# mvenouziou/Boosted_DETR

Hardware: AMD Instinct MI355X
Metric: images/sec training step (fwd+matcher+loss+bwd), 640x640 N=100 (higher is better)
Workload: dtype f32 (conv/GEMM products as 3 split-f16 [fwd] / split-bf16 [grad] MFMA products, f32 accumulate)

## Files before the change

### boosted_detr_amd/csrc/gemm_common.h

```cpp
#pragma once
#include "common.h"
#include <type_traits>

namespace bdgemm {

enum { ST_STORE = 0, ST_ACCUM = 1, ST_ATOMIC = 2 };
enum { AR_FP32 = 0, AR_BF16X3 = 1, AR_FP16X3 = 2, AR_P16_F16 = 3, AR_P16_BF16 = 4, AR_BF16X6 = 5 };

struct GemmParams {
    int I, J, R;
    int nb1;
    int splitk, r_chunk;
    int tiles_i, tiles_j;
    float* c; int64_t ldc, sc0, sc1;
    const float* bias; float alpha; int act; int mode;
    float* stat_sum; float* stat_sq;
    int vec_store;
    int rowmap;
    int rm_OW, rm_OHOW, rm_H, rm_W, rm_stride;
    int rm_off;
    int ngroups;
    const float* ga[4]; const float* gb[4]; float* gc[4]; const float* gbias[4]; int gI[4];
    const float* bnb_y; const float* bnb_mean; const float* bnb_rstd; const float* bnb_gamma; const float* bnb_beta;
    int bnb_relu; float* bnb_sum_g; float* bnb_sum_gx;
    const unsigned long long* bnb_mask;
    const float* bnb2_y; const float* bnb2_mean; const float* bnb2_rstd; float* bnb2_sum_gx;
    const unsigned long long* acc_mask;
    const float* acc_src; int acc_H, acc_W;
    int b_f16;
#ifdef BDETR_SGEMM_DIAG
    int dbg;
#endif
};

#ifdef BDETR_SGEMM_DIAG
#define BDETR_DBG(g, bits) (((g).dbg & (bits)) != 0)
#else
#define BDETR_DBG(g, bits) false
#endif

inline void init_params(GemmParams& g) {
    g = GemmParams{};
    g.nb1 = 1; g.splitk = 1; g.alpha = 1.f; g.mode = ST_STORE;
}

__device__ __forceinline__ float apply_act(float v, int act) {
    if (act == BDETR_ACT_RELU) return fmaxf(v, 0.f);
    if (act == BDETR_ACT_TANH) return tanhf(v);
    return v;
}

__device__ __forceinline__ int xcd_tile(int bid, int nwg) {
    const int q = nwg >> 3, r = nwg & 7, xcd = bid & 7, idx = bid >> 3;
    return (xcd < r ? xcd * (q + 1) : r * (q + 1) + (xcd - r) * q) + idx;
}

template <int BM, int BN, int WM, int WN>
__device__ __forceinline__ void gemm_load_bias(const GemmParams& g, int j0, float (&bias_pre)[BN / WN / 32]) {
    const int tid = threadIdx.x, lane = tid & 63, wave = tid >> 6, wn = wave % WN;
#pragma unroll
    for (int b = 0; b < BN / WN / 32; ++b) {
        const int j = j0 + wn * (BN / WN) + b * 32 + (lane & 31);
        bias_pre[b] = (g.bias != nullptr && j < g.J) ? g.bias[j] : 0.f;
    }
}

template <int BM, int BN, int WM, int WN>
__device__ __forceinline__ void gemm_bias_act_stats(f32x16 (&acc)[BM / WM / 32][BN / WN / 32], const GemmParams& g, int tile_i, int i0, int j0,
                                                    const float* bias_pre = nullptr) {
    constexpr int WTM = BM / WM, WTN = BN / WN, TM = WTM / 32, TN = WTN / 32;
    int tid = threadIdx.x;
    asm volatile("" : "+v"(tid));
    const int lane = tid & 63, wave = __builtin_amdgcn_readfirstlane(tid >> 6);
    const int wm = wave / WN, wn = wave % WN, li = lane & 31, lh = lane >> 5;
    auto bias_act_stats = [&](auto act_c) {
        constexpr int ACT = decltype(act_c)::value;
#pragma unroll
        for (int b = 0; b < TN; ++b) {
            const int j = j0 + wn * WTN + b * 32 + li;
            const bool jok = j < g.J;
            const float bias = bias_pre != nullptr ? bias_pre[b] : ((g.bias != nullptr && jok) ? g.bias[j] : 0.f);
            float csum = 0.f, csq = 0.f;
#pragma unroll
            for (int a = 0; a < TM; ++a) {
#pragma unroll
                for (int e = 0; e < 16; ++e) {
                    const int i = i0 + wm * WTM + a * 32 + (e & 3) + 8 * (e >> 2) + 4 * lh;
                    const float v = apply_act(g.alpha * acc[a][b][e] + bias, ACT);
                    acc[a][b][e] = v;
                    const float vs = (i < g.I && jok) ? v : 0.f;
                    csum += vs; csq += vs * vs;
                }
            }
            if (g.stat_sum != nullptr) {
                csum += __shfl_xor(csum, 32, 64);
                csq += __shfl_xor(csq, 32, 64);
                if (lh == 0 && jok) {
                    const int64_t chunk = (int64_t)tile_i * WM + wm;
                    g.stat_sum[chunk * g.J + j] = csum;
                    g.stat_sq[chunk * g.J + j] = csq;
                }
            }
        }
    };
    if (g.act == BDETR_ACT_NONE) {
        if (g.bias != nullptr || g.alpha != 1.f || g.stat_sum != nullptr) bias_act_stats(std::integral_constant<int, BDETR_ACT_NONE>{});
    } else if (g.act == BDETR_ACT_RELU) bias_act_stats(std::integral_constant<int, BDETR_ACT_RELU>{});
    else bias_act_stats(std::integral_constant<int, BDETR_ACT_TANH>{});
}

__device__ __forceinline__ unsigned mask_bits4(const unsigned long long* mask, int64_t i) {
    const unsigned long long* w = mask + (i >> 6) * 4;
    const int b = (int)(i & 63);
    return (unsigned)((w[0] >> b) & 1ull) | ((unsigned)((w[1] >> b) & 1ull) << 1) | ((unsigned)((w[2] >> b) & 1ull) << 2) | ((unsigned)((w[3] >> b) & 1ull) << 3);
}

template <int BM, int BN, int WM, int WN, int NT, int LDS_FLOATS, bool MASKED_VARIANTS = false, bool BNB2_ONLY = false, bool COMPACT_ONLY = false>
__device__ __forceinline__ void gemm_epilogue(f32x16 (&acc)[BM / WM / 32][BN / WN / 32], const GemmParams& g, float* lds,
                                              int tile_i, int i0, int j0, float* cbase, const float* bias_pre = nullptr) {
    constexpr int WTM = BM / WM, WTN = BN / WN, TM = WTM / 32, TN = WTN / 32;
    const int tid = threadIdx.x, lane = tid & 63, wave = tid >> 6;
    const int wm = wave / WN, wn = wave % WN, li = lane & 31, lh = lane >> 5;
    auto out_row = [&](int i) -> int64_t {
        if (!g.rowmap) return i;
        int n = i / g.rm_OHOW; int rem = i - n * g.rm_OHOW;
        int oh = rem / g.rm_OW; int ow = rem - oh * g.rm_OW;
        return ((int64_t)n * g.rm_H + (int64_t)oh * g.rm_stride) * g.rm_W + (int64_t)ow * g.rm_stride + g.rm_off;
    };
    gemm_bias_act_stats<BM, BN, WM, WN>(acc, g, tile_i, i0, j0, bias_pre);

    if (g.vec_store && g.mode != ST_ATOMIC) {
        constexpr bool PAD = BM * (BN + 4) <= LDS_FLOATS;
        constexpr int CLD = PAD ? BN + 4 : BN;
        static_assert(BM * CLD <= LDS_FLOATS, "epilogue tile must fit in the staging LDS");
        constexpr bool SWZ = !PAD && BN % 64 == 0;
        __syncthreads();
#pragma unroll
        for (int a = 0; a < TM; ++a)
#pragma unroll
            for (int b = 0; b < TN; ++b)
#pragma unroll
                for (int e = 0; e < 16; ++e)
                    lds[(wm * WTM + a * 32 + (e & 3) + 8 * (e >> 2) + 4 * lh) * CLD + ((wn * WTN + b * 32 + li) ^ (SWZ ? lh << 5 : 0))] = acc[a][b][e];
        __syncthreads();
        constexpr int V_PER_ROW = BN / 4, RSTEP = NT / V_PER_ROW, ITERS = BM / RSTEP;
        static_assert(NT % V_PER_ROW == 0 && BM % RSTEP == 0, "a thread keeps one column group and a fixed row stride");
        static_assert(!SWZ || RSTEP % 8 == 0, "the swizzle bit of a thread's rows must not change between iterations");
        const int c4 = tid % V_PER_ROW, r0 = tid / V_PER_ROW;
        const int jc = j0 + 4 * c4;
        const bool jok = jc < g.J;
        const float* lrow = lds + r0 * CLD + ((4 * c4) ^ (SWZ ? ((r0 >> 2) & 1) << 5 : 0));
        auto vec_out = [&](auto rowmap_c, auto accum_c, auto bnb_c, auto masked_c, auto bnb2_c, auto compact_c) {
            constexpr bool ROWMAP = decltype(rowmap_c)::value, ACCUM = decltype(accum_c)::value, BNB = decltype(bnb_c)::value, MASKED = decltype(masked_c)::value;
            constexpr bool BNB2 = decltype(bnb2_c)::value;
            constexpr bool COMPACT = decltype(compact_c)::value;
            static_assert(!COMPACT || (ACCUM && MASKED && !ROWMAP && !BNB2), "the compact old gradient rides the masked accumulate");
            static_assert(!BNB2 || (BNB && ACCUM && MASKED), "the second BatchNorm rides the masked accumulate with masked sums");
            constexpr int NPART = (ACCUM && BNB) ? (BNB2 && ITERS % 4 == 0 ? 4 : 2) : 1, PIT = ITERS / NPART;
            static_assert(ITERS % NPART == 0, "the tile splits into equal parts");
            f32x4 bnv[BNB ? 6 : 1];
            f32x4 bn2[BNB2 ? 3 : 1];
            if constexpr (BNB2) {
                bn2[0] = f32x4{0, 0, 0, 0}; bn2[1] = f32x4{0, 0, 0, 0}; bn2[2] = f32x4{0, 0, 0, 0};
                if (jok) { bn2[0] = *reinterpret_cast<const f32x4*>(g.bnb2_mean + jc); bn2[1] = *reinterpret_cast<const f32x4*>(g.bnb2_rstd + jc); }
            }
            if constexpr (BNB) {
#pragma unroll
                for (int q = 0; q < 6; ++q) bnv[q] = f32x4{0, 0, 0, 0};
                if (jok) {
                    bnv[0] = *reinterpret_cast<const f32x4*>(g.bnb_mean + jc); bnv[1] = *reinterpret_cast<const f32x4*>(g.bnb_rstd + jc);
                    bnv[2] = *reinterpret_cast<const f32x4*>(g.bnb_gamma + jc); bnv[3] = *reinterpret_cast<const f32x4*>(g.bnb_beta + jc);
                }
            }
#pragma unroll
// ... 145 lines not shown
```

### boosted_detr_amd/csrc/sgemm.hip

```cpp
#include "gemm_common.h"
#include "p16.h"
#include <stdlib.h>
#include <string.h>
#include <type_traits>
#include <utility>

using namespace bdgemm;

namespace {

constexpr int BK = 32;
constexpr unsigned OOB = 0xFFFFFFF0u;
constexpr unsigned NUM_RECORDS = 0xFFFFFF00u;

typedef __bf16 bf16x8 __attribute__((ext_vector_type(8)));
typedef _Float16 f16x8 __attribute__((ext_vector_type(8)));
typedef unsigned int u32x4 __attribute__((ext_vector_type(4)));
typedef unsigned int u32x2 __attribute__((ext_vector_type(2)));
typedef short s16x4 __attribute__((ext_vector_type(4)));
typedef __attribute__((address_space(3))) void lds_void;

__device__ __forceinline__ __amdgpu_buffer_rsrc_t make_rsrc(const void* p, unsigned records = NUM_RECORDS) {
    const unsigned long long a = reinterpret_cast<unsigned long long>(p);
    const unsigned lo = __builtin_amdgcn_readfirstlane((unsigned)a), hi = __builtin_amdgcn_readfirstlane((unsigned)(a >> 32));
// ... 63 lines not shown
    static __device__ __forceinline__ Col col(const Op& op, int x0, int slot, int x_lim, int r_uni, int lane_row) {
        const int r_first = r_uni + lane_row;
        Col c; c.ok = x0 + 8 * (slot >> 1) < x_lim; c.r = r_first;
        c.off = (unsigned)r_first * op.ld * 4u + (unsigned)x0 * 4u + 16u * (unsigned)slot; return c;
    }
    template <int RPI> static __device__ __forceinline__ unsigned voff(const Op&, const Col& c, int r_lim) { return (c.ok && c.r < r_lim) ? c.off : OOB; }
    static __device__ __forceinline__ void advance(const Op& op, Col& c) { c.r += BK; c.off += (unsigned)BK * op.ld * 4u; }
};
struct XXPatch {
    using Op = PPatch;
    using Row = int; using Step = int;
    static __device__ __forceinline__ unsigned records(const Op&) { return NUM_RECORDS; }
    struct Col { int r, oh, ow, ih, iw; unsigned off; bool ok; };
    static __device__ __forceinline__ Col col(const Op& op, int x0, int slot, int x_lim, int r_uni, int lane_row) {
        const int r_first = r_uni + lane_row;
        Col c; const int x = x0 + 8 * (slot >> 1);
        c.ok = x < x_lim; c.r = r_first;
        const int tap = x / op.C, ch = x - tap * op.C;
        const int tr = tap / op.S, ts = tap - tr * op.S;
        const int ohw = op.OH * op.OW;
        const int n = r_first / ohw, rem = r_first - n * ohw;
        c.oh = rem / op.OW; c.ow = rem - c.oh * op.OW;
        c.ih = c.oh * op.stride - op.pad + tr; c.iw = c.ow * op.stride - op.pad + ts;
        c.off = ((unsigned)(n * op.H * op.W) + (unsigned)(c.ih * op.W + c.iw)) * (unsigned)op.C * 4u + (unsigned)ch * 4u + 16u * (unsigned)(slot & 1);
        return c;
    }
    template <int RPI> static __device__ __forceinline__ unsigned voff(const Op& op, const Col& c, int r_lim) {
        const bool ok = c.ok && c.r < r_lim && (unsigned)c.ih < (unsigned)op.H && (unsigned)c.iw < (unsigned)op.W;
        return ok ? c.off : OOB;
    }
    static __device__ __forceinline__ void advance(const Op& op, Col& c) {
        c.r += BK;
        c.ow += op.d_ow; c.oh += op.d_oh; c.iw += op.d_ow * op.stride; c.ih += op.d_oh * op.stride; c.off += op.k_step;
        const bool w = c.ow >= op.OW;
        c.ow -= w ? op.OW : 0; c.oh += w ? 1 : 0; c.iw -= w ? op.OW * op.stride : 0; c.ih += w ? op.stride : 0; c.off += w ? op.k_wrap_ow : 0u;
        if (op.single_wrap) {
            const bool v = c.oh >= op.OH;
            c.oh -= v ? op.OH : 0; c.ih -= v ? op.OH * op.stride : 0; c.off += v ? op.k_wrap_oh : 0u;
        } else {
            while (c.oh >= op.OH) { c.oh -= op.OH; c.ih -= op.OH * op.stride; c.off += op.k_wrap_oh; }
        }
    }
};

__device__ __forceinline__ int xx_swz(int r) { return ((r & 1) << 3) | ((r >> 1) & 1); }

#if defined(BDETR_SGEMM_STAMPS) && defined(BDETR_SGEMM_DIAG)
__device__ unsigned long long g_stamps[64];
#endif

constexpr int lds_bytes_for(int bm, int bn, int ns) { return ns * (bm + bn) * 128 > bm * bn * 4 ? ns * (bm + bn) * 128 : bm * bn * 4; }

enum { EPI_PLAIN = 0, EPI_ROWMAP = 1, EPI_VEC = 8, EPI_BNB2 = 16, EPI_COMPACT = 32 };
template <int BM, int BN, int WM, int WN, bool STATS = true, int EPI = EPI_ROWMAP>
__device__ __forceinline__ void direct_epilogue(f32x16 (&acc)[BM / WM / 32][BN / WN / 32], const GemmParams& g, int tile_i, int i0, int j0, const float* bias_pre) {
    constexpr int WTM = BM / WM, WTN = BN / WN, TM = WTM / 32, TN = WTN / 32;
    constexpr unsigned FAR = 0x80000000u;
    if constexpr (STATS) gemm_bias_act_stats<BM, BN, WM, WN>(acc, g, tile_i, i0, j0, bias_pre);
    int tid = threadIdx.x;
    asm volatile("" : "+v"(tid));
    const int lane = tid & 63, wave = __builtin_amdgcn_readfirstlane(tid >> 6);
    const int wm = wave / WN, wn = wave % WN, li = lane & 31, lh = lane >> 5;

    const unsigned ldc4 = (unsigned)g.ldc * 4u;
    const int rows_here = min(BM, g.I - i0);
    const int jl = j0 + wn * WTN + li;
    auto tile_rsrc = [&](const float* base) {
        const unsigned long long p = reinterpret_cast<unsigned long long>(base) + (unsigned long long)i0 * ldc4;
        const unsigned lo = __builtin_amdgcn_readfirstlane((unsigned)p), hi = __builtin_amdgcn_readfirstlane((unsigned)(p >> 32));
        return __builtin_amdgcn_make_buffer_rsrc(reinterpret_cast<void*>(((unsigned long long)hi << 32) | lo), 0,
                                                 __builtin_amdgcn_readfirstlane(rows_here * (int)ldc4), 0x00020000);
    };
    unsigned vcol[TN];
#pragma unroll
    for (int b = 0; b < TN; ++b) vcol[b] = jl + b * 32 < g.J ? (unsigned)(wm * WTM + 4 * lh) * ldc4 + (unsigned)(jl + b * 32) * 4u : FAR;
    auto for_rows = [&](auto&& f) {
        unsigned ro = 0;
#pragma unroll
        for (int a = 0; a < TM; ++a)
#pragma unroll
            for (int e = 0; e < 16; ++e) { f(a, e, ro); ro += (e & 3) == 3 ? 5u * ldc4 : ldc4; }
    };

    if constexpr ((EPI & EPI_ROWMAP) != 0) if (g.rowmap) {
        const __amdgpu_buffer_rsrc_t rsC = make_rsrc(g.c);
        const int i = i0 + wm * WTM + (lane % WTM);
        const int n = i / g.rm_OHOW, rem = i - n * g.rm_OHOW, oh = rem / g.rm_OW, ow = rem - oh * g.rm_OW;
        const unsigned rmap = i < g.I ? (unsigned)((n * g.rm_H + oh * g.rm_stride) * g.rm_W + ow * g.rm_stride + g.rm_off) * ldc4 : OOB;
        const bool accum = g.mode == ST_ACCUM;
#pragma unroll
        for (int a = 0; a < TM; ++a)
#pragma unroll
            for (int e = 0; e < 16; ++e) {
                const unsigned ro = (unsigned)__shfl((int)rmap, a * 32 + (e & 3) + 8 * (e >> 2) + 4 * lh, 64);
#pragma unroll
                for (int b = 0; b < TN; ++b) {
                    const unsigned vo = (ro != OOB && jl + b * 32 < g.J) ? ro + (unsigned)(jl + b * 32) * 4u : OOB;
                    float v = acc[a][b][e];
                    if (accum) v += __uint_as_float(__builtin_amdgcn_raw_buffer_load_b32(rsC, vo, 0, 0));
                    if (!BDETR_DBG(g, 1)) __builtin_amdgcn_raw_buffer_store_b32(__float_as_uint(v), rsC, vo, 0, 0);
                }
            }
        return;
    }

    const __amdgpu_buffer_rsrc_t rsC = tile_rsrc(g.c);
// ... 2 lines not shown
#pragma unroll
        for (int b = 0; b < TN; ++b) {
            const float v = acc[a][b][e];
            __builtin_amdgcn_raw_buffer_store_b32(__float_as_uint(v), rsC, vcol[b] + ro, 0, 0);
        }
    });
}

template <int BM, int BN, int WM, int WN>
__device__ __forceinline__ void atomic_epilogue(f32x16 (&acc)[BM / WM / 32][BN / WN / 32], const GemmParams& g, int i0, int j0) {
    constexpr int WTM = BM / WM, WTN = BN / WN, TM = WTM / 32, TN = WTN / 32;
    constexpr unsigned FAR = 0x80000000u;
    const int tid = threadIdx.x, lane = tid & 63, wave = __builtin_amdgcn_readfirstlane(tid >> 6);
    const int wm = wave / WN, wn = wave % WN, li = lane & 31, lh = lane >> 5;
    const unsigned ldc4 = (unsigned)g.ldc * 4u;
    const int rows_here = min(BM, g.I - i0);
    const unsigned long long p = reinterpret_cast<unsigned long long>(g.c) + (unsigned long long)i0 * ldc4;
    const unsigned lo = __builtin_amdgcn_readfirstlane((unsigned)p), hi = __builtin_amdgcn_readfirstlane((unsigned)(p >> 32));
    const __amdgpu_buffer_rsrc_t rsC = __builtin_amdgcn_make_buffer_rsrc(reinterpret_cast<void*>(((unsigned long long)hi << 32) | lo), 0,
                                                                         __builtin_amdgcn_readfirstlane(rows_here * (int)ldc4), 0x00020000);
    unsigned vcol[TN];
#pragma unroll
    for (int b = 0; b < TN; ++b) {
        const int j = j0 + wn * WTN + b * 32 + li;
        vcol[b] = j < g.J ? (unsigned)(wm * WTM + 4 * lh) * ldc4 + (unsigned)j * 4u : FAR;
    }
    unsigned ro = 0;
#pragma unroll
    for (int a = 0; a < TM; ++a)
#pragma unroll
        for (int e = 0; e < 16; ++e) {
#pragma unroll
            for (int b = 0; b < TN; ++b) {
                const float v = g.alpha * acc[a][b][e];
                __builtin_amdgcn_raw_ptr_buffer_atomic_fadd_f32(v, rsC, vcol[b] + ro, 0, 0);
            }
            ro += (e & 3) == 3 ? 5u * ldc4 : ldc4;
            asm volatile("" : "+v"(ro));
        }
}

constexpr int default_occ(int bm, int bn, int wm, int wn, int ns) { return (wm * wn == 4 && 2 * lds_bytes_for(bm, bn, ns) <= 160 * 1024) ? 2 : (wm * wn == 8 ? 2 : 1); }

template <int BM, int BN, int WM, int WN, int NS, class LA, class LB, bool XX, bool F16, bool PP = false, int OCC = default_occ(BM, BN, WM, WN, NS), int EPI = EPI_ROWMAP>
__global__ __launch_bounds__(WM * WN * 64, OCC)
void sgemm_kernel(typename LA::Op opa, typename LB::Op opb, GemmParams g)
{
    constexpr int NW = WM * WN, NT = NW * 64;
    constexpr int WTM = BM / WM, WTN = BN / WN, TM = WTM / 32, TN = WTN / 32;
    static_assert(TM >= 1 && TN >= 1, "wave tile must hold at least one 32x32 MFMA tile");
    constexpr int A_BYTES = BM * 128, B_BYTES = BN * 128, STAGE_BYTES = A_BYTES + B_BYTES;
    constexpr int NIA = A_BYTES / 1024 / NW, NIB = B_BYTES / 1024 / NW;
    static_assert(NIA >= 1 && NIB >= 1 && NIA * NW * 1024 == A_BYTES && NIB * NW * 1024 == B_BYTES, "tile / wave count mismatch");
    constexpr int LDS_BYTES = lds_bytes_for(BM, BN, NS);
    static_assert(NS >= 2 && NS <= 4 && LDS_BYTES <= 160 * 1024, "LDS budget");
    static_assert(BK == 32, "fragment helpers assume two 16-deep MFMA steps per stage");
    __shared__ __attribute__((aligned(16))) unsigned char lds[LDS_BYTES];

    const int tid = threadIdx.x;
    const int lane = tid & 63;
    const int wave = __builtin_amdgcn_readfirstlane(tid >> 6);
    const int wm = wave / WN, wn = wave % WN;
    const int li = lane & 31, lh = lane >> 5;

    constexpr bool PERSIST = !PP && !XX && std::is_same_v<LA, RRDense> && (EPI & EPI_VEC) == 0;
    static_assert(PP ? (NS == 3 && NW == 8) : NS == 2, "the plain loops are written for a two-stage ring, the ping-pong loop for three stages and 8 waves");
    const int nwg = g.tiles_i * g.tiles_j;
    const int total = PERSIST ? nwg : nwg * (int)gridDim.z;
    int vb = PERSIST ? (int)blockIdx.x : (int)(blockIdx.z * nwg + blockIdx.x);
    int tile_i, i0, j0, zz;
    auto locate = [&](int v) {
        const int lin = xcd_tile(v, total);
        zz = lin / nwg;
        const int wg = lin - zz * nwg;
        tile_i = wg / g.tiles_j;
        const int tile_j = wg - tile_i * g.tiles_j;
        i0 = tile_i * BM; j0 = tile_j * BN;
    };
    locate(vb);

    int r_begin = 0, r_end = g.R;
    if (g.splitk > 1) { r_begin = zz * g.r_chunk; r_end = min(g.R, r_begin + g.r_chunk); }

    const __amdgpu_buffer_rsrc_t rsA = make_rsrc(opa.p, LA::records(opa));
    const __amdgpu_buffer_rsrc_t rsB = make_rsrc(opb.p, LB::records(opb));

    typename LA::Row rowA[NIA]; typename LB::Row rowB[NIB]; typename LA::Col colA[NIA]; typename LB::Col colB[NIB];
    int rrA[NIA], rrB[NIB];
    static_assert(XX || NW % 2 == 0, "one source chunk per lane needs an even wave count");
    const int qsrc = (lane & 7) ^ (((wave & 1) << 2) | (lane >> 4));
    const int klimA = min(r_end, (int)opa.cols) - 8 * (qsrc >> 1), klimB = min(r_end, (int)opb.cols) - 8 * (qsrc >> 1);
    typename LA::Step stA; typename LB::Step stB;
    auto setup_rows = [&]() {
        if constexpr (!XX) {
#pragma unroll
            for (int t = 0; t < NIA; ++t) {
                const int x = (t * NW + wave) * 8 + (lane >> 3);
                rowA[t] = LA::row(opa, i0 + x, qsrc);
            }
#pragma unroll
            for (int t = 0; t < NIB; ++t) {
                const int x = (t * NW + wave) * 8 + (lane >> 3);
                rowB[t] = LB::row(opb, j0 + x, qsrc);
            }
            stA = LA::step_init(opa, r_begin); stB = LB::step_init(opb, r_begin);
        }
    };
    setup_rows();
    if constexpr (XX) {
        constexpr int SA = BM / 4, SB = BN / 4;
        static_assert(SA >= 16 && SB >= 16 && SA <= 64 && SB <= 64, "XX tiles: 64 <= BX <= 256");
#pragma unroll
        for (int t = 0; t < NIA; ++t) {
            const int ru = (t * NW + wave) * (64 / SA), r = ru + lane / SA;
            rrA[t] = r;
            colA[t] = LA::col(opa, i0, (lane % SA) ^ xx_swz(r), opa.cols, r_begin + ru, lane / SA);
        }
#pragma unroll
        for (int t = 0; t < NIB; ++t) {
            const int ru = (t * NW + wave) * (64 / SB), r = ru + lane / SB;
            rrB[t] = r;
            colB[t] = LB::col(opb, j0, (lane % SB) ^ xx_swz(r), opb.cols, r_begin + ru, lane / SB);
        }
    }

    auto issue_one = [&](int buf, int r0, auto l_c) {
        constexpr int l = decltype(l_c)::value;
        unsigned char* sa = lds + buf * STAGE_BYTES;
        if constexpr (l < NIA) {
            constexpr int t = l;
            unsigned vo;
            if constexpr (!XX) vo = LA::voff(opa, rowA[t], stA, r0, klimA);
            else               vo = LA::template voff<256 / BM>(opa, colA[t], min(r_end, opa.rows));
            __builtin_amdgcn_raw_ptr_buffer_load_lds(rsA, (lds_void*)(sa + (t * NW + wave) * 1024), 16, (int)vo, 0, 0, 0);
        } else {
            constexpr int t = l - NIA;
            unsigned vo;
            if constexpr (!XX) vo = LB::voff(opb, rowB[t], stB, r0, klimB);
            else               vo = LB::template voff<256 / BN>(opb, colB[t], min(r_end, opb.rows));
            __builtin_amdgcn_raw_ptr_buffer_load_lds(rsB, (lds_void*)(sa + A_BYTES + (t * NW + wave) * 1024), 16, (int)vo, 0, 0, 0);
        }
    };
    constexpr int NLOAD = NIA + NIB;
    auto issue_all = [&](int buf, int r0) {
        if (BDETR_DBG(g, 16)) return;
        [&]<int... L>(std::integer_sequence<int, L...>) { (issue_one(buf, r0, std::integral_constant<int, L>{}), ...); }(std::make_integer_sequence<int, NLOAD>{});
        if constexpr (!XX) { LA::step_next(opa, stA); LB::step_next(opb, stB); }
        else {
#pragma unroll
            for (int t = 0; t < NIA; ++t) LA::advance(opa, colA[t]);
#pragma unroll
            for (int t = 0; t < NIB; ++t) LB::advance(opb, colB[t]);
        }
    };

    f32x16 acc[TM][TN];
    auto zero_acc = [&]() {
        float z = 0.f;
        asm volatile("" : "+v"(z));
#pragma unroll
        for (int a = 0; a < TM; ++a)
#pragma unroll
            for (int b = 0; b < TN; ++b)
#pragma unroll
                for (int e = 0; e < 16; ++e) acc[a][b][e] = z;
    };
    zero_acc();

    auto frag_rr = [&](const unsigned char* tile, int x, int ks, u32x4& hi, u32x4& lo) {
        const int s = (2 * (2 * ks + lh)) ^ ((x >> 1) & 7);
        const unsigned char* p = tile + x * 128;
        hi = *reinterpret_cast<const u32x4*>(p + s * 16);
        lo = *reinterpret_cast<const u32x4*>(p + (s ^ 1) * 16);
    };
    auto frag_xx = [&](const unsigned char* tile, auto rowbytes_c, int xw, auto ks_c, u32x4& hi, u32x4& lo) {
        constexpr int rowbytes = decltype(rowbytes_c)::value, ks = decltype(ks_c)::value;
        const int g16 = (lane >> 4) & 1, q = (lane >> 2) & 3, p = lane & 3;
        const int unit = (xw + 16 * g16 + 4 * p) >> 3;
        const int r0 = 8 * lh + q;
        const int sl = (2 * unit) ^ xx_swz(r0);
        const unsigned base = (unsigned)(size_t)(__attribute__((address_space(3))) const unsigned char*)tile + (unsigned)(r0 * rowbytes + 8 * (p & 1));
        const unsigned ah = base + (unsigned)(sl * 16), al = base + (unsigned)((sl ^ 1) * 16);
        u32x2 h0, h1, l0, l1;
        constexpr int o0 = ks * 16 * rowbytes, o1 = o0 + 4 * rowbytes;
        static_assert(o1 < 65536, "ds offset field");
        asm volatile("ds_read_b64_tr_b16 %0, %1 offset:%2" : "=v"(h0) : "v"(ah), "n"(o0));
        asm volatile("ds_read_b64_tr_b16 %0, %1 offset:%2" : "=v"(l0) : "v"(al), "n"(o0));
        asm volatile("ds_read_b64_tr_b16 %0, %1 offset:%2" : "=v"(h1) : "v"(ah), "n"(o1));
        asm volatile("ds_read_b64_tr_b16 %0, %1 offset:%2" : "=v"(l1) : "v"(al), "n"(o1));
        hi[0] = h0[0]; hi[1] = h0[1]; hi[2] = h1[0]; hi[3] = h1[1];
        lo[0] = l0[0]; lo[1] = l0[1]; lo[2] = l1[0]; lo[3] = l1[1];
    };
    auto frag_wait = [&](u32x4 (&ah)[TM], u32x4 (&al)[TM], u32x4 (&bh)[TN], u32x4 (&bl)[TN]) {
        if constexpr (XX) {
            static_assert(TM <= 2 && TN <= 2, "frag_wait ties at most 2 + 2 fragments");
            if constexpr (TM == 2 && TN == 2)
                asm volatile("s_waitcnt lgkmcnt(0)" : "+v"(ah[0]), "+v"(al[0]), "+v"(ah[1]), "+v"(al[1]), "+v"(bh[0]), "+v"(bl[0]), "+v"(bh[1]), "+v"(bl[1]));
            else if constexpr (TM == 2 && TN == 1)
                asm volatile("s_waitcnt lgkmcnt(0)" : "+v"(ah[0]), "+v"(al[0]), "+v"(ah[1]), "+v"(al[1]), "+v"(bh[0]), "+v"(bl[0]));
            else if constexpr (TM == 1 && TN == 2)
                asm volatile("s_waitcnt lgkmcnt(0)" : "+v"(ah[0]), "+v"(al[0]), "+v"(bh[0]), "+v"(bl[0]), "+v"(bh[1]), "+v"(bl[1]));
            else
                asm volatile("s_waitcnt lgkmcnt(0)" : "+v"(ah[0]), "+v"(al[0]), "+v"(bh[0]), "+v"(bl[0]));
        }
    };
    auto load_frags = [&](int buf, auto ks_c, u32x4 (&ah)[TM], u32x4 (&al)[TM], u32x4 (&bh)[TN], u32x4 (&bl)[TN]) {
        constexpr int ks = decltype(ks_c)::value;
        const unsigned char* tA = lds + buf * STAGE_BYTES;
        const unsigned char* tB = tA + A_BYTES;
#pragma unroll
        for (int a = 0; a < TM; ++a) {
            if constexpr (!XX) frag_rr(tA, wm * WTM + a * 32 + li, ks, ah[a], al[a]);
            else               frag_xx(tA, std::integral_constant<int, BM * 4>{}, wm * WTM + a * 32, ks_c, ah[a], al[a]);
        }
#pragma unroll
        for (int b = 0; b < TN; ++b) {
            if constexpr (!XX) frag_rr(tB, wn * WTN + b * 32 + li, ks, bh[b], bl[b]);
            else               frag_xx(tB, std::integral_constant<int, BN * 4>{}, wn * WTN + b * 32, ks_c, bh[b], bl[b]);
        }
    };
    auto mfma_ks = [&](const u32x4 (&ah)[TM], const u32x4 (&al)[TM], const u32x4 (&bh)[TN], const u32x4 (&bl)[TN]) {
#pragma unroll
        for (int a = 0; a < TM; ++a)
#pragma unroll
            for (int b = 0; b < TN; ++b) {
                if constexpr (F16) {
#define H8(v) __builtin_bit_cast(f16x8, v)
                    acc[a][b] = __builtin_amdgcn_mfma_f32_32x32x16_f16(H8(al[a]), H8(bh[b]), acc[a][b], 0, 0, 0);
                    acc[a][b] = __builtin_amdgcn_mfma_f32_32x32x16_f16(H8(ah[a]), H8(bl[b]), acc[a][b], 0, 0, 0);
                    acc[a][b] = __builtin_amdgcn_mfma_f32_32x32x16_f16(H8(ah[a]), H8(bh[b]), acc[a][b], 0, 0, 0);
#undef H8
                } else {
#define BF8(v) __builtin_bit_cast(bf16x8, v)
                    acc[a][b] = __builtin_amdgcn_mfma_f32_32x32x16_bf16(BF8(al[a]), BF8(bh[b]), acc[a][b], 0, 0, 0);
                    acc[a][b] = __builtin_amdgcn_mfma_f32_32x32x16_bf16(BF8(ah[a]), BF8(bl[b]), acc[a][b], 0, 0, 0);
                    acc[a][b] = __builtin_amdgcn_mfma_f32_32x32x16_bf16(BF8(ah[a]), BF8(bh[b]), acc[a][b], 0, 0, 0);
#undef BF8
                }
            }
    };
    auto f16pair_to_bf16pair = [&](u32x4& hi, u32x4& lo) {
        const unsigned hw[4] = {hi[0], hi[1], hi[2], hi[3]}, lw[4] = {lo[0], lo[1], lo[2], lo[3]};
#pragma unroll
        for (int w = 0; w < 4; ++w) {
            const p16_f32x2 hf = __builtin_convertvector(__builtin_bit_cast(p16_f16x2, hw[w]), p16_f32x2);
            const p16_f32x2 lf = __builtin_convertvector(__builtin_bit_cast(p16_f16x2, lw[w]), p16_f32x2);
            unsigned bh_, bl_;
            p16_split2_bf16(hf[0] + lf[0], hf[1] + lf[1], bh_, bl_);
            hi[w] = bh_; lo[w] = bl_;
        }
    };
    auto kstep = [&](int buf) {
        if (BDETR_DBG(g, 8)) return;
        auto half = [&](auto ks_c) {
            u32x4 ah[TM], al[TM], bh[TN], bl[TN];
            load_frags(buf, ks_c, ah, al, bh, bl);
            frag_wait(ah, al, bh, bl);
            if constexpr (XX && !F16) {
                if (g.b_f16) {
#pragma unroll
                    for (int b = 0; b < TN; ++b) f16pair_to_bf16pair(bh[b], bl[b]);
                }
            }
            mfma_ks(ah, al, bh, bl);
        };
        static_assert(BK / 16 == 2, "two 16-deep halves per stage");
        half(std::integral_constant<int, 0>{});
        half(std::integral_constant<int, 1>{});
    };

    if constexpr (PP) {
        constexpr int NLOAD_ = NIA + NIB;
        const int nk = (r_end - r_begin + BK - 1) / BK;
        float bias_pre[TN];
        gemm_load_bias<BM, BN, WM, WN>(g, j0, bias_pre);
        const bool grpY = wave >= NW / 2;
        u32x4 fah[2][TM], fal[2][TM], fbh[2][TN], fbl[2][TN];
        auto read_all = [&](auto buf_c) {
            constexpr int buf = decltype(buf_c)::value;
            load_frags(buf, std::integral_constant<int, 0>{}, fah[0], fal[0], fbh[0], fbl[0]);
            load_frags(buf, std::integral_constant<int, 1>{}, fah[1], fal[1], fbh[1], fbl[1]);
            frag_wait(fah[0], fal[0], fbh[0], fbl[0]);
            frag_wait(fah[1], fal[1], fbh[1], fbl[1]);
            if constexpr (XX && !F16) {
                if (g.b_f16) {
#pragma unroll
                    for (int ks = 0; ks < 2; ++ks)
#pragma unroll
                        for (int b = 0; b < TN; ++b) f16pair_to_bf16pair(fbh[ks][b], fbl[ks][b]);
                }
            }
        };
        auto mfma_step = [&]() {
            asm volatile("s_waitcnt lgkmcnt(0)" ::: "memory");
            __builtin_amdgcn_sched_barrier(0);
            __builtin_amdgcn_s_setprio(1);
#pragma unroll
            for (int ks = 0; ks < 2; ++ks) mfma_ks(fah[ks], fal[ks], fbh[ks], fbl[ks]);
            __builtin_amdgcn_s_setprio(0);
            __builtin_amdgcn_sched_barrier(0);
        };
        if (nk > 0) issue_all(0, r_begin);
        if (nk > 1) issue_all(1, r_begin + BK);
        if (nk > 1) asm volatile("s_waitcnt vmcnt(%0)\n\ts_barrier" :: "n"(NLOAD_) : "memory");
        else        asm volatile("s_waitcnt vmcnt(0)\n\ts_barrier" ::: "memory");
        if (!grpY) read_all(std::integral_constant<int, 0>{});
        auto step = [&](int t, auto b0_c, auto b1_c, auto b2_c) {
            constexpr int b2 = decltype(b2_c)::value;
            if (!grpY) {
                mfma_step();
                asm volatile("s_waitcnt vmcnt(0)\n\ts_barrier" ::: "memory");
            } else {
                read_all(b0_c);
                if (t + 2 < nk) {
                    issue_all(b2, r_begin + (t + 2) * BK);
                    asm volatile("s_waitcnt vmcnt(%0)\n\ts_barrier" :: "n"(NLOAD_) : "memory");
                } else {
                    asm volatile("s_waitcnt vmcnt(0)\n\ts_barrier" ::: "memory");
                }
            }
            if (grpY) {
                mfma_step();
            } else {
                if (t + 1 < nk) read_all(b1_c);
                if (t + 2 < nk) issue_all(b2, r_begin + (t + 2) * BK);
            }
            asm volatile("s_barrier" ::: "memory");
        };
        using I0 = std::integral_constant<int, 0>; using I1 = std::integral_constant<int, 1>; using I2 = std::integral_constant<int, 2>;
        for (int t = 0; t < nk; t += 3) {
            step(t, I0{}, I1{}, I2{});
            if (t + 1 < nk) step(t + 1, I1{}, I2{}, I0{});
            if (t + 2 < nk) step(t + 2, I2{}, I0{}, I1{});
        }
        if (XX && g.mode == ST_ATOMIC && g.bias == nullptr && g.act == BDETR_ACT_NONE && g.stat_sum == nullptr && !g.rowmap && g.ldc * 4 * BM < (1ll << 31)) {
            atomic_epilogue<BM, BN, WM, WN>(acc, g, i0, j0);
            return;
        }
        gemm_epilogue<BM, BN, WM, WN, NT, LDS_BYTES / 4>(acc, g, reinterpret_cast<float*>(lds), tile_i, i0, j0, g.c + (g.splitk > 1 ? (int64_t)zz * g.sc0 : 0), bias_pre);
    } else if constexpr (PERSIST) {
        const int nk = BDETR_DBG(g, 2) ? 0 : (g.R + BK - 1) / BK;
        auto prefetch = [&]() { if (nk > 0) issue_all(0, 0); if (nk > 1) issue_all(1, BK); };
        prefetch();
        for (;;) {
            float bias_pre[TN];
            gemm_load_bias<BM, BN, WM, WN>(g, j0, bias_pre);
            for (int kt = 0; kt < nk; kt += 2) {
                asm volatile("s_waitcnt vmcnt(0)\n\ts_barrier" ::: "memory");
                if (kt >= 1 && kt + 1 < nk) issue_all(1, (kt + 1) * BK);
                kstep(0);
                if (kt + 1 < nk) {
                    asm volatile("s_waitcnt vmcnt(0)\n\ts_barrier" ::: "memory");
                    if (kt + 2 < nk) issue_all(0, (kt + 2) * BK);
                    kstep(1);
                }
            }
            gemm_bias_act_stats<BM, BN, WM, WN>(acc, g, tile_i, i0, j0, bias_pre);
            const int e_tile_i = tile_i, e_i0 = i0, e_j0 = j0;
            const int nvb = vb + (int)gridDim.x;
            const bool more = nvb < total;
            if (more) { locate(nvb); setup_rows(); }
            asm volatile("s_barrier" ::: "memory");
            if (more) prefetch();
            direct_epilogue<BM, BN, WM, WN, false, EPI>(acc, g, e_tile_i, e_i0, e_j0, bias_pre);
            if (!more) break;
            vb = nvb;
            zero_acc();
        }
    } else {
        const int nk = BDETR_DBG(g, 2) ? 0 : (r_end - r_begin + BK - 1) / BK;
        float bias_pre[TN];
        gemm_load_bias<BM, BN, WM, WN>(g, j0, bias_pre);
        if (nk > 0) issue_all(0, r_begin);
#if defined(BDETR_SGEMM_STAMPS) && defined(BDETR_SGEMM_DIAG)
        if (BDETR_DBG(g, 32) && blockIdx.x == 1 && blockIdx.z == 0 && wave == 0) {
            unsigned long long st[48];
            auto stamp = [&](int i) { unsigned long long t; asm volatile("s_memtime %0\n\ts_waitcnt lgkmcnt(0)" : "=s"(t) :: "memory"); st[i] = t; };
#pragma unroll
            for (int kt = 0; kt < 12; ++kt) {
                if (kt < nk) {
                    asm volatile("s_waitcnt vmcnt(0)" ::: "memory"); stamp(4 * kt);
                    asm volatile("s_barrier" ::: "memory"); stamp(4 * kt + 1);
                    if (kt + 1 < nk) issue_all((kt + 1) & 1, r_begin + (kt + 1) * BK);
                    stamp(4 * kt + 2);
                    kstep(kt & 1);
                    stamp(4 * kt + 3);
                }
            }
            for (int kt = 12; kt < nk; ++kt) {
                asm volatile("s_waitcnt vmcnt(0)\n\ts_barrier" ::: "memory");
                if (kt + 1 < nk) issue_all((kt + 1) & 1, r_begin + (kt + 1) * BK);
                kstep(kt & 1);
// ... 2 lines not shown
        } else
#endif
        for (int kt = 0; kt < nk; kt += 2) {
            asm volatile("s_waitcnt vmcnt(0)\n\ts_barrier" ::: "memory");
            if (kt + 1 < nk) issue_all(1, r_begin + (kt + 1) * BK);
            kstep(0);
            if (kt + 1 < nk) {
                asm volatile("s_waitcnt vmcnt(0)\n\ts_barrier" ::: "memory");
                if (kt + 2 < nk) issue_all(0, r_begin + (kt + 2) * BK);
                kstep(1);
            }
        }
        if (XX && g.mode == ST_ATOMIC && g.bias == nullptr && g.act == BDETR_ACT_NONE && g.stat_sum == nullptr && !g.rowmap && g.ldc * 4 * BM < (1ll << 31)) {
            atomic_epilogue<BM, BN, WM, WN>(acc, g, i0, j0);
            return;
        }
        gemm_epilogue<BM, BN, WM, WN, NT, LDS_BYTES / 4, (EPI & EPI_VEC) != 0, (EPI & EPI_BNB2) != 0, (EPI & EPI_COMPACT) != 0>(acc, g, reinterpret_cast<float*>(lds), tile_i, i0, j0, g.c + (g.splitk > 1 ? (int64_t)zz * g.sc0 : 0), bias_pre);
    }
}

enum { T_128x128 = 0, T_128x64 = 1, T_64x64 = 2, T_PP256x128 = 3, T_PP256x64 = 4, T_COUNT = 5 };
const int TILE_BM[T_COUNT] = {128, 128, 64, 256, 256};
const int TILE_BN[T_COUNT] = {128, 64, 64, 128, 64};
const int TILE_WM[T_COUNT] = {2, 2, 2, 4, 4};
constexpr int DENSE128_WM = 2;
int tile_wm(int tile, bool dense) { return (dense && tile == T_128x128) ? DENSE128_WM : TILE_WM[tile]; }

int forced_tile() {
    static int forced = -2;
    if (forced == -2) {
        forced = -1;
        if (const char* e = getenv("BDETR_STILE")) {
            const char* names[T_COUNT] = {"128x128", "128x64", "64x64", "pp256x128", "pp256x64"};
            for (int t = 0; t < T_COUNT; ++t) if (!strcmp(e, names[t])) forced = t;
            if (!strcmp(e, "pp")) forced = T_PP256x128;
        }
    }
    return forced;
}

int choose_tile(int64_t I, int64_t J, int64_t z, bool pp_ok = false) {
    int forced = forced_tile();
    if (forced >= T_PP256x128) {
        const bool patch = pp_ok;
        if (!patch) forced = -1;
        else return J % 128 == 0 ? T_PP256x128 : (J % 64 == 0 ? T_PP256x64 : T_128x64);
    }
    if (forced >= 0) return (J < 64 || (TILE_BN[forced] == 128 && J < 128)) ? T_64x64 : forced;
    const int64_t cus = num_cus();
    auto tiles = [&](int bm, int bn) { return cdiv64(I, bm) * cdiv64(J, bn) * z; };
    if (J % 128 == 0 && tiles(128, 128) >= cus) return T_128x128;
    if (tiles(128, 64) >= cus) return T_128x64;
    return T_64x64;
}

template <int BM, int BN, int WM, int WN, int NS, class LA, class LB, bool XX, bool F16, bool PP = false, int OCC = default_occ(BM, BN, WM, WN, NS)>
int launch_cfg(const typename LA::Op& a, const typename LB::Op& b, GemmParams g, int zdim, hipStream_t st, int kind) {
    g.tiles_i = (int)cdiv64(g.I, BM);
    g.tiles_j = (int)cdiv64(g.J, BN);
    dim3 grid(g.tiles_i * g.tiles_j, 1, zdim);
    g.vec_store = (g.J % 4 == 0) && (g.ldc % 4 == 0) && aligned16(g.c);
#ifdef BDETR_SGEMM_DIAG
    static int dbg = -1;
    if (dbg < 0) { const char* e = getenv("BDETR_SGEMM_DBG"); dbg = e ? atoi(e) : 0; }
    g.dbg = dbg;
    if (dbg & 4) g.vec_store = 0;
#endif
    const bool prof = g_prof_on;
    if (prof) prof_begin(st, 2.0 * (double)g.I * (double)g.J * (double)g.R, g.I, g.J, g.R, zdim, BM, BN * 10 + NS,
                         (F16 ? AR_P16_F16 : AR_P16_BF16) * 10000 + kind);
    if constexpr (!PP && !XX && std::is_same_v<LA, RRDense>) {
        auto go = [&](auto epi_c) {
            hipLaunchKernelGGL((sgemm_kernel<BM, BN, WM, WN, NS, LA, LB, XX, F16, PP, OCC, decltype(epi_c)::value>), grid, dim3(WM * WN * 64), 0, st, a, b, g);
            if (prof) prof_end(st);
            return bdetr_launch_status("sgemm");
        };
        BDETR_CHECK_ARG(zdim == 1 && g.splitk == 1, "sgemm: the dense 1x1 kernels take no split-K / batch dimension");
        if (!g.rowmap && (g.mode == ST_ACCUM || g.bnb_y != nullptr)) {
            BDETR_CHECK_ARG(g.vec_store, "sgemm: accumulate / fused BatchNorm-backward sums need 16-byte aligned C rows and J %% 4 == 0");
            BDETR_CHECK_ARG(g.acc_mask == nullptr || g.mode == ST_ACCUM, "sgemm: acc_mask without accumulate");
            BDETR_CHECK_ARG(g.bnb_mask == nullptr || (g.acc_mask != nullptr && g.bnb_y != nullptr), "sgemm: a bit-mask ReLU decision comes with a masked accumulate");
            if (g.acc_src != nullptr) {
                BDETR_CHECK_ARG(g.acc_mask != nullptr && g.bnb2_y == nullptr && g.acc_H > 0 && g.acc_W > 0 && g.acc_H % 2 == 0 && g.acc_W % 2 == 0 && g.I % (g.acc_H * g.acc_W) == 0,
                                "sgemm: a compact old gradient needs the masked accumulate, an even map that divides the rows, and no second BatchNorm");
                return go(std::integral_constant<int, EPI_VEC | EPI_COMPACT>{});
            }
            if (g.bnb2_y != nullptr) return go(std::integral_constant<int, EPI_VEC | EPI_BNB2>{});
            return go(std::integral_constant<int, EPI_VEC>{});
        }
        BDETR_CHECK_ARG(g.acc_mask == nullptr && g.bnb_y == nullptr, "sgemm: masks / fused sums are not available with a row map");
        static int resident = 0;
        if (resident == 0) {
            int occ = 0;
            if (hipOccupancyMaxActiveBlocksPerMultiprocessor(&occ, sgemm_kernel<BM, BN, WM, WN, NS, LA, LB, XX, F16, PP, OCC, EPI_ROWMAP>, WM * WN * 64, 0) != hipSuccess || occ < 1) occ = 1;
            resident = occ * num_cus() / 8 * 8;
            if (resident < 8) resident = 8;
        }
        if ((int)grid.x > resident) grid.x = resident;
        if (!g.rowmap) return go(std::integral_constant<int, EPI_PLAIN>{});
        return go(std::integral_constant<int, EPI_ROWMAP>{});
    }
    hipLaunchKernelGGL((sgemm_kernel<BM, BN, WM, WN, NS, LA, LB, XX, F16, PP, OCC>), grid, dim3(WM * WN * 64), 0, st, a, b, g);
    if (prof) prof_end(st);
    return bdetr_launch_status("sgemm");
}

template <class LA, class LB, bool XX, bool F16>
int launch_any(const typename LA::Op& a, const typename LB::Op& b, const GemmParams& g, int zdim, hipStream_t st, int kind, int tile) {
    switch (tile) {
        case T_128x128:
            if constexpr (!XX && std::is_same_v<LA, RRDense> && DENSE128_WM == 4) return launch_cfg<128, 128, 4, 2, 2, LA, LB, XX, F16, false, 4>(a, b, g, zdim, st, kind);
            else return launch_cfg<128, 128, 2, 2, 2, LA, LB, XX, F16>(a, b, g, zdim, st, kind);
        case T_128x64:     return launch_cfg<128, 64, 2, 2, 2, LA, LB, XX, F16>(a, b, g, zdim, st, kind);
        case T_PP256x128:
            if constexpr (std::is_same_v<LA, RRPatch> && !F16) return launch_cfg<256, 128, 4, 2, 3, LA, LB, XX, F16, true>(a, b, g, zdim, st, kind);
            else return launch_cfg<128, 128, 2, 2, 2, LA, LB, XX, F16>(a, b, g, zdim, st, kind);
        case T_PP256x64:
            if constexpr (std::is_same_v<LA, RRPatch> && !F16) return launch_cfg<256, 64, 4, 2, 3, LA, LB, XX, F16, true>(a, b, g, zdim, st, kind);
            else return launch_cfg<128, 64, 2, 2, 2, LA, LB, XX, F16>(a, b, g, zdim, st, kind);
        default:           return launch_cfg<64, 64, 2, 2, 2, LA, LB, XX, F16>(a, b, g, zdim, st, kind);
    }
}

constexpr int64_t MAX_OPERAND_ELEMS = (int64_t)(NUM_RECORDS / 4) - (4 << 20);
bool span_ok(int64_t elems) { return elems >= 0 && elems <= MAX_OPERAND_ELEMS; }

int check_conv(const bdetr_conv_desc* d, const char* who) {
    BDETR_CHECK_ARG(d != nullptr, "%s: null desc", who);
    BDETR_CHECK_ARG(d->N > 0 && d->H > 0 && d->W > 0 && d->C > 0 && d->K > 0 && d->R > 0 && d->S > 0 && d->stride > 0 && d->pad >= 0,
                    "%s: bad conv geometry", who);
    BDETR_CHECK_ARG(d->OH == (d->H + 2 * d->pad - d->R) / d->stride + 1 && d->OW == (d->W + 2 * d->pad - d->S) / d->stride + 1,
                    "%s: OH/OW inconsistent with geometry", who);
    BDETR_CHECK_ARG(d->C % 8 == 0 && d->K % 8 == 0, "%s: the P16 layout needs channel counts that are multiples of 8 (C=%d K=%d)", who, d->C, d->K);
    BDETR_CHECK_ARG((d->R == 1 && d->S == 1) || d->C % BK == 0, "%s: kernels larger than 1x1 need C %% %d == 0 (C=%d)", who, BK, d->C);
    BDETR_CHECK_ARG(d->R * d->S <= 32 && (int64_t)d->R * d->S * d->C <= 16384 && d->C <= 16384 && d->K <= 16384, "%s: at most 32 taps and rows of at most 16,384 elements", who);
    BDETR_CHECK_ARG((int64_t)d->N * d->OH * d->OW < (1LL << 31) && (int64_t)d->R * d->S * d->C < (1LL << 31) && (int64_t)d->N * d->H * d->W < (1LL << 31),
                    "%s: problem too large", who);
    BDETR_CHECK_ARG(span_ok((int64_t)d->N * d->H * d->W * d->C) && span_ok((int64_t)d->N * d->OH * d->OW * d->K) && span_ok((int64_t)d->K * d->R * d->S * d->C),
                    "%s: a tensor spans 4 GB or more (the loaders use 32-bit buffer offsets); use a smaller per-GPU batch", who);
    return 0;
// ... 294 lines not shown
```

Before: 644.7.

## Add A-resident dense GEMM kernel reusing LDS A panel across column tiles

Adds a variant of the dense 1x1 backward GEMM with vectorised epilogue for short reductions (R up to 256). It keeps the whole A row panel resident in LDS and loops over a group of column tiles, streaming only B through a two-slot ring. The aim is to stop reloading A for every output column tile and to cut per-tile launch/prologue cost. The trade-off is more LDS per block, and so lower occupancy when the panel is large. It also adds barrier-serialised load/compute steps and extra template instantiations. It is on by default through an environment toggle.

```diff
diff --git a/boosted_detr_amd/csrc/gemm_common.h b/boosted_detr_amd/csrc/gemm_common.h
--- a/boosted_detr_amd/csrc/gemm_common.h
+++ b/boosted_detr_amd/csrc/gemm_common.h
@@ -28,6 +28,7 @@
     const unsigned long long* acc_mask;
     const float* acc_src; int acc_H, acc_W;
     int b_f16;
+    int res_tpg;
 #ifdef BDETR_SGEMM_DIAG
     int dbg;
 #endif
@@ -115,11 +116,13 @@
     return (unsigned)((w[0] >> b) & 1ull) | ((unsigned)((w[1] >> b) & 1ull) << 1) | ((unsigned)((w[2] >> b) & 1ull) << 2) | ((unsigned)((w[3] >> b) & 1ull) << 3);
 }
 
-template <int BM, int BN, int WM, int WN, int NT, int LDS_FLOATS, bool MASKED_VARIANTS = false, bool BNB2_ONLY = false, bool COMPACT_ONLY = false>
+template <int BM, int BN, int WM, int WN, int NT, int LDS_FLOATS, bool MASKED_VARIANTS = false, bool BNB2_ONLY = false, bool COMPACT_ONLY = false, bool LAUNDER = false>
 __device__ __forceinline__ void gemm_epilogue(f32x16 (&acc)[BM / WM / 32][BN / WN / 32], const GemmParams& g, float* lds,
                                               int tile_i, int i0, int j0, float* cbase, const float* bias_pre = nullptr) {
     constexpr int WTM = BM / WM, WTN = BN / WN, TM = WTM / 32, TN = WTN / 32;
-    const int tid = threadIdx.x, lane = tid & 63, wave = tid >> 6;
+    int tid_ = threadIdx.x;
+    if constexpr (LAUNDER) asm volatile("" : "+v"(tid_));
+    const int tid = tid_, lane = tid & 63, wave = tid >> 6;
     const int wm = wave / WN, wn = wave % WN, li = lane & 31, lh = lane >> 5;
     auto out_row = [&](int i) -> int64_t {
         if (!g.rowmap) return i;
diff --git a/boosted_detr_amd/csrc/sgemm.hip b/boosted_detr_amd/csrc/sgemm.hip
--- a/boosted_detr_amd/csrc/sgemm.hip
+++ b/boosted_detr_amd/csrc/sgemm.hip
@@ -139,6 +139,11 @@
 constexpr int lds_bytes_for(int bm, int bn, int ns) { return ns * (bm + bn) * 128 > bm * bn * 4 ? ns * (bm + bn) * 128 : bm * bn * 4; }
 
 enum { EPI_PLAIN = 0, EPI_ROWMAP = 1, EPI_VEC = 8, EPI_BNB2 = 16, EPI_COMPACT = 32 };
+constexpr int EPI_RES(int nkp) { return nkp << 8; }
+constexpr int res_ksteps(int epi) { return (epi >> 8) & 15; }
+constexpr int res_scratch_bytes(int bm, int bn, int panel) {
+    return panel + bm * (bn + 4) * 4 <= 160 * 1024 ? bm * (bn + 4) * 4 : (bm * bn * 4 > 2 * bn * 128 ? bm * bn * 4 : 2 * bn * 128);
+}
 template <int BM, int BN, int WM, int WN, bool STATS = true, int EPI = EPI_ROWMAP>
 __device__ __forceinline__ void direct_epilogue(f32x16 (&acc)[BM / WM / 32][BN / WN / 32], const GemmParams& g, int tile_i, int i0, int j0, const float* bias_pre) {
     constexpr int WTM = BM / WM, WTN = BN / WN, TM = WTM / 32, TN = WTN / 32;
@@ -247,7 +252,11 @@
     constexpr int A_BYTES = BM * 128, B_BYTES = BN * 128, STAGE_BYTES = A_BYTES + B_BYTES;
     constexpr int NIA = A_BYTES / 1024 / NW, NIB = B_BYTES / 1024 / NW;
     static_assert(NIA >= 1 && NIB >= 1 && NIA * NW * 1024 == A_BYTES && NIB * NW * 1024 == B_BYTES, "tile / wave count mismatch");
-    constexpr int LDS_BYTES = lds_bytes_for(BM, BN, NS);
+    constexpr int NKP = res_ksteps(EPI);
+    constexpr bool RES = NKP > 0;
+    static_assert(!RES || ((EPI & EPI_VEC) != 0 && !PP && !XX && std::is_same_v<LA, RRDense> && std::is_same_v<LB, RRDense>), "the A-resident kernel is a dense RR EPI_VEC kernel");
+    constexpr int RES_SCRATCH = RES ? res_scratch_bytes(BM, BN, NKP * A_BYTES) : 0;
+    constexpr int LDS_BYTES = RES ? NKP * A_BYTES + RES_SCRATCH : lds_bytes_for(BM, BN, NS);
     static_assert(NS >= 2 && NS <= 4 && LDS_BYTES <= 160 * 1024, "LDS budget");
     static_assert(BK == 32, "fragment helpers assume two 16-deep MFMA steps per stage");
     __shared__ __attribute__((aligned(16))) unsigned char lds[LDS_BYTES];
@@ -319,9 +328,8 @@
         }
     }
 
-    auto issue_one = [&](int buf, int r0, auto l_c) {
+    auto issue_one = [&](unsigned char* sa, unsigned char* sb, int r0, auto l_c) {
         constexpr int l = decltype(l_c)::value;
-        unsigned char* sa = lds + buf * STAGE_BYTES;
         if constexpr (l < NIA) {
             constexpr int t = l;
             unsigned vo;
@@ -333,13 +341,14 @@
             unsigned vo;
             if constexpr (!XX) vo = LB::voff(opb, rowB[t], stB, r0, klimB);
             else               vo = LB::template voff<256 / BN>(opb, colB[t], min(r_end, opb.rows));
-            __builtin_amdgcn_raw_ptr_buffer_load_lds(rsB, (lds_void*)(sa + A_BYTES + (t * NW + wave) * 1024), 16, (int)vo, 0, 0, 0);
+            __builtin_amdgcn_raw_ptr_buffer_load_lds(rsB, (lds_void*)(sb + (t * NW + wave) * 1024), 16, (int)vo, 0, 0, 0);
         }
     };
     constexpr int NLOAD = NIA + NIB;
     auto issue_all = [&](int buf, int r0) {
         if (BDETR_DBG(g, 16)) return;
-        [&]<int... L>(std::integer_sequence<int, L...>) { (issue_one(buf, r0, std::integral_constant<int, L>{}), ...); }(std::make_integer_sequence<int, NLOAD>{});
+        unsigned char* sa = lds + buf * STAGE_BYTES;
+        [&]<int... L>(std::integer_sequence<int, L...>) { (issue_one(sa, sa + A_BYTES, r0, std::integral_constant<int, L>{}), ...); }(std::make_integer_sequence<int, NLOAD>{});
         if constexpr (!XX) { LA::step_next(opa, stA); LB::step_next(opb, stB); }
         else {
 #pragma unroll
@@ -399,10 +408,8 @@
                 asm volatile("s_waitcnt lgkmcnt(0)" : "+v"(ah[0]), "+v"(al[0]), "+v"(bh[0]), "+v"(bl[0]));
         }
     };
-    auto load_frags = [&](int buf, auto ks_c, u32x4 (&ah)[TM], u32x4 (&al)[TM], u32x4 (&bh)[TN], u32x4 (&bl)[TN]) {
+    auto load_frags_at = [&](const unsigned char* tA, const unsigned char* tB, auto ks_c, u32x4 (&ah)[TM], u32x4 (&al)[TM], u32x4 (&bh)[TN], u32x4 (&bl)[TN]) {
         constexpr int ks = decltype(ks_c)::value;
-        const unsigned char* tA = lds + buf * STAGE_BYTES;
-        const unsigned char* tB = tA + A_BYTES;
 #pragma unroll
         for (int a = 0; a < TM; ++a) {
             if constexpr (!XX) frag_rr(tA, wm * WTM + a * 32 + li, ks, ah[a], al[a]);
@@ -413,6 +420,10 @@
             if constexpr (!XX) frag_rr(tB, wn * WTN + b * 32 + li, ks, bh[b], bl[b]);
             else               frag_xx(tB, std::integral_constant<int, BN * 4>{}, wn * WTN + b * 32, ks_c, bh[b], bl[b]);
         }
+    };
+    auto load_frags = [&](int buf, auto ks_c, u32x4 (&ah)[TM], u32x4 (&al)[TM], u32x4 (&bh)[TN], u32x4 (&bl)[TN]) {
+        const unsigned char* tA = lds + buf * STAGE_BYTES;
+        load_frags_at(tA, tA + A_BYTES, ks_c, ah, al, bh, bl);
     };
     auto mfma_ks = [&](const u32x4 (&ah)[TM], const u32x4 (&al)[TM], const u32x4 (&bh)[TN], const u32x4 (&bl)[TN]) {
 #pragma unroll
@@ -445,11 +456,11 @@
             hi[w] = bh_; lo[w] = bl_;
         }
     };
-    auto kstep = [&](int buf) {
+    auto kstep_at = [&](const unsigned char* tA, const unsigned char* tB) {
         if (BDETR_DBG(g, 8)) return;
         auto half = [&](auto ks_c) {
             u32x4 ah[TM], al[TM], bh[TN], bl[TN];
-            load_frags(buf, ks_c, ah, al, bh, bl);
+            load_frags_at(tA, tB, ks_c, ah, al, bh, bl);
             frag_wait(ah, al, bh, bl);
             if constexpr (XX && !F16) {
                 if (g.b_f16) {
@@ -463,6 +474,7 @@
         half(std::integral_constant<int, 0>{});
         half(std::integral_constant<int, 1>{});
     };
+    auto kstep = [&](int buf) { const unsigned char* tA = lds + buf * STAGE_BYTES; kstep_at(tA, tA + A_BYTES); };
 
     if constexpr (PP) {
         constexpr int NLOAD_ = NIA + NIB;
@@ -533,6 +545,44 @@
             return;
         }
         gemm_epilogue<BM, BN, WM, WN, NT, LDS_BYTES / 4>(acc, g, reinterpret_cast<float*>(lds), tile_i, i0, j0, g.c + (g.splitk > 1 ? (int64_t)zz * g.sc0 : 0), bias_pre);
+    } else if constexpr (RES) {
+        const int nk = BDETR_DBG(g, 2) ? 0 : (g.R + BK - 1) / BK;
+        const int tpg = g.res_tpg, ngrp = (g.tiles_j + tpg - 1) / tpg;
+        const int lin = xcd_tile((int)blockIdx.x, g.tiles_i * ngrp);
+        tile_i = lin / ngrp;
+        const int tj0 = (lin - tile_i * ngrp) * tpg, tj1 = min(g.tiles_j, tj0 + tpg);
+        i0 = tile_i * BM;
+        unsigned char* const ring = lds + NKP * A_BYTES;
+        for (int tj = tj0; tj < tj1; ++tj) {
+            j0 = tj * BN;
+            setup_rows();
+            const bool fill = tj == tj0;
+            auto issue = [&](int kt, int buf) {
+                if (BDETR_DBG(g, 16)) return;
+                unsigned char* sa = lds + kt * A_BYTES;
+                unsigned char* sb = ring + buf * B_BYTES;
+                if (fill) [&]<int... L>(std::integer_sequence<int, L...>) { (issue_one(sa, sb, kt * BK, std::integral_constant<int, L>{}), ...); }(std::make_integer_sequence<int, NIA>{});
+                [&]<int... L>(std::integer_sequence<int, L...>) { (issue_one(sa, sb, kt * BK, std::integral_constant<int, NIA + L>{}), ...); }(std::make_integer_sequence<int, NIB>{});
+            };
+            float bias_pre[TN];
+            gemm_load_bias<BM, BN, WM, WN>(g, j0, bias_pre);
+            if (nk > 0) issue(0, 0);
+            for (int kt = 0; kt < nk; kt += 2) {
+                asm volatile("s_waitcnt vmcnt(0)\n\ts_barrier" ::: "memory");
+                if (kt + 1 < nk) issue(kt + 1, 1);
+                kstep_at(lds + kt * A_BYTES, ring);
+                if (kt + 1 < nk) {
+                    asm volatile("s_waitcnt vmcnt(0)\n\ts_barrier" ::: "memory");
+                    if (kt + 2 < nk) issue(kt + 2, 0);
+                    kstep_at(lds + (kt + 1) * A_BYTES, ring + B_BYTES);
+                }
+            }
+            gemm_epilogue<BM, BN, WM, WN, NT, RES_SCRATCH / 4, true, (EPI & EPI_BNB2) != 0, (EPI & EPI_COMPACT) != 0, true>(acc, g, reinterpret_cast<float*>(ring), tile_i, i0, j0, g.c, bias_pre);
+            if (tj + 1 < tj1) {
+                asm volatile("s_waitcnt lgkmcnt(0)\n\ts_barrier" ::: "memory");
+                zero_acc();
+            }
+        }
     } else if constexpr (PERSIST) {
         const int nk = BDETR_DBG(g, 2) ? 0 : (g.R + BK - 1) / BK;
         auto prefetch = [&]() { if (nk > 0) issue_all(0, 0); if (nk > 1) issue_all(1, BK); };
@@ -641,6 +691,22 @@
     if (J % 128 == 0 && tiles(128, 128) >= cus) return T_128x128;
     if (tiles(128, 64) >= cus) return T_128x64;
     return T_64x64;
+}
+
+int resident_cols(const GemmParams& g, int occ) {
+    static int on = -1, groups = 0;
+    if (on < 0) {
+        const char* e = getenv("BDETR_P16_RESIDENT"); on = e ? atoi(e) != 0 : 1;
+        const char* f = getenv("BDETR_P16_RESIDENT_GROUPS"); groups = f ? atoi(f) : 0;
+    }
+    if (!on || g.R > 8 * BK || g.tiles_j < 2) return 0;
+    int ngrp = groups;
+    if (ngrp <= 0) {
+        const int slots = occ * num_cus();
+        ngrp = g.tiles_i >= slots ? 1 : (slots + g.tiles_i - 1) / g.tiles_i;
+    }
+    if (ngrp > g.tiles_j) ngrp = g.tiles_j;
+    return (g.tiles_j + ngrp - 1) / ngrp;
 }
 
 template <int BM, int BN, int WM, int WN, int NS, class LA, class LB, bool XX, bool F16, bool PP = false, int OCC = default_occ(BM, BN, WM, WN, NS)>
@@ -669,12 +735,33 @@
             BDETR_CHECK_ARG(g.vec_store, "sgemm: accumulate / fused BatchNorm-backward sums need 16-byte aligned C rows and J %% 4 == 0");
             BDETR_CHECK_ARG(g.acc_mask == nullptr || g.mode == ST_ACCUM, "sgemm: acc_mask without accumulate");
             BDETR_CHECK_ARG(g.bnb_mask == nullptr || (g.acc_mask != nullptr && g.bnb_y != nullptr), "sgemm: a bit-mask ReLU decision comes with a masked accumulate");
-            if (g.acc_src != nullptr) {
+            if (g.acc_src != nullptr)
                 BDETR_CHECK_ARG(g.acc_mask != nullptr && g.bnb2_y == nullptr && g.acc_H > 0 && g.acc_W > 0 && g.acc_H % 2 == 0 && g.acc_W % 2 == 0 && g.I % (g.acc_H * g.acc_W) == 0,
                                 "sgemm: a compact old gradient needs the masked accumulate, an even map that divides the rows, and no second BatchNorm");
-                return go(std::integral_constant<int, EPI_VEC | EPI_COMPACT>{});
-            }
-            if (g.bnb2_y != nullptr) return go(std::integral_constant<int, EPI_VEC | EPI_BNB2>{});
+            const int epi = g.acc_src != nullptr ? EPI_VEC | EPI_COMPACT : (g.bnb2_y != nullptr ? EPI_VEC | EPI_BNB2 : EPI_VEC);
+            if constexpr (BM == 128 && BN == 64 && WM == 2 && WN == 2 && NS == 2 && !F16) {
+                const int nk = (g.R + BK - 1) / BK, nkp = nk <= 2 ? 2 : (nk <= 4 ? 4 : 8), occ = nkp == 2 ? 2 : 1;
+                if (const int tpg = resident_cols(g, occ)) {
+                    g.res_tpg = tpg;
+                    grid.x = g.tiles_i * ((g.tiles_j + tpg - 1) / tpg);
+                    auto res = [&](auto epi_c, auto nkp_c) {
+                        constexpr int E = decltype(epi_c)::value | EPI_RES(decltype(nkp_c)::value);
+                        hipLaunchKernelGGL((sgemm_kernel<BM, BN, WM, WN, NS, LA, LB, XX, F16, PP, decltype(nkp_c)::value == 2 ? 2 : 1, E>), grid, dim3(WM * WN * 64), 0, st, a, b, g);
+                        if (prof) prof_end(st);
+                        return bdetr_launch_status("sgemm");
+                    };
+                    auto by_epi = [&](auto nkp_c) {
+                        if (epi == (EPI_VEC | EPI_COMPACT)) return res(std::integral_constant<int, EPI_VEC | EPI_COMPACT>{}, nkp_c);
+                        if (epi == (EPI_VEC | EPI_BNB2)) return res(std::integral_constant<int, EPI_VEC | EPI_BNB2>{}, nkp_c);
+                        return res(std::integral_constant<int, EPI_VEC>{}, nkp_c);
+                    };
+                    if (nkp == 2) return by_epi(std::integral_constant<int, 2>{});
+                    if (nkp == 4) return by_epi(std::integral_constant<int, 4>{});
+                    return by_epi(std::integral_constant<int, 8>{});
+                }
+            }
+            if (epi == (EPI_VEC | EPI_COMPACT)) return go(std::integral_constant<int, EPI_VEC | EPI_COMPACT>{});
+            if (epi == (EPI_VEC | EPI_BNB2)) return go(std::integral_constant<int, EPI_VEC | EPI_BNB2>{});
             return go(std::integral_constant<int, EPI_VEC>{});
         }
         BDETR_CHECK_ARG(g.acc_mask == nullptr && g.bnb_y == nullptr, "sgemm: masks / fused sums are not available with a row map");
```

Result: slower. 219.0, median of 2 (-66.0%).
